# marcinp7/music-style-transfer

Hardware: AMD Instinct MI355X
Metric: style-transfer opt iters/sec (higher is better)
Workload: dtype f32; 1 GPU; one 30 s clip per GPU (BASELINE.json configs[1]): piano-roll C=4,R=16,T=4 (+percussion), full widths (980325 params), fwd+loss+bwd every step, Adam+StepLR every iter_size steps; clips_per_gpu=1, iter_size=2, hip_graph=True, graphs=one joint graph, accumulation=2 concurrent streams, launches_per_pass=71, parallelism=single GPU

## Files before the change

### music-style-transfer_amd/csrc/loss_optim.hip

```cpp
#include "mst_common.h"

#define LOSS_MAXBLK 256
#define NP_SUMS 7
#define N_TAPE_IN 16
#define SAVED_J 0
#define EPS_DIV 1e-7f

int64_t mst_loss_scratch_floats(void) { return 2 * LOSS_MAXBLK * 8 + 64; }

template <int NFEAT>
__device__ __forceinline__ void note_terms(const float* p, const float* t, float* acc) {
    const float pv = p[1], tv = t[1];
    const float m = tv > 0.f ? 1.f : 0.f;
    acc[0] += fminf(pv, tv);
    acc[1] += fmaxf(pv - tv, 0.f);
    acc[2] += fmaxf(tv - pv, 0.f);
    const float dv = tv - pv;
    acc[3] += dv * dv * m;
    const float dd = (p[0] - fminf(t[0], 6.f)) / 6.f;
    acc[4] += dd * dd * m;
    if (NFEAT == 5) {
        float bce = 0.f;
#pragma unroll
        for (int a = 2; a < 5; ++a) {
// ... 112 lines not shown
        o.acc = d_div(in[5], d_cmul(NM, 3.f));
        if (normalize) o.acc = d_tanh(o.acc);
        o.total = d_qmean3(o.dur, o.acc, nv);
    } else {
        o.acc = dl(0.f, 0.f);
        o.total = d_qmean2(o.dur, nv);
    }
    return o;
}

__global__ __launch_bounds__(64) void loss_tail_kernel(const float* scratch, int nblk_p, int nblk_u, int has_u,
                                                       const float* il, const float* it, int ni,
                                                       const float* mlg, const float* mt,
                                                       const float* bp, const float* bt, int normalize,
                                                       float* losses, float* saved, LossBatch lb,
                                                       float* gl_onehot, float* losses_out) {
    __shared__ float sums[N_TAPE_IN];
    const int tid = threadIdx.x;
    {
        const int64_t k = blockIdx.y;
        scratch += k * lb.tmp; il += k * lb.ws; it += k * lb.ws; mlg += k * lb.ws; mt += k * lb.ws; bp += k * lb.ws;
        bt += k * lb.ws; losses += k * lb.ws; saved += k * lb.ws;
        if (gl_onehot) gl_onehot += k * lb.ws;
        if (losses_out) losses_out += k * MST_N_LOSSES;
    }
    {
        float sp[8] = {0.f, 0.f, 0.f, 0.f, 0.f, 0.f, 0.f, 0.f}, su[8] = {0.f, 0.f, 0.f, 0.f, 0.f, 0.f, 0.f, 0.f};
        typedef float row4 __attribute__((ext_vector_type(4), aligned(4)));
        const row4* rp = reinterpret_cast<const row4*>(scratch);
        const row4* ru = reinterpret_cast<const row4*>(scratch + LOSS_MAXBLK * 8);
        const int nbu = has_u ? nblk_u : 0;
        for (int q = tid; q < nblk_p; q += 64) {
            const row4 x = rp[2 * q], y = rp[2 * q + 1];
            sp[0] += x.x; sp[1] += x.y; sp[2] += x.z; sp[3] += x.w; sp[4] += y.x; sp[5] += y.y; sp[6] += y.z;
        }
        for (int q = tid; q < nbu; q += 64) {
            const row4 x = ru[2 * q], y = ru[2 * q + 1];
            su[0] += x.x; su[1] += x.y; su[2] += x.z; su[3] += x.w; su[4] += y.x; su[5] += y.y; su[6] += y.z;
        }
// ... 11 lines not shown
    for (int j = tid; j < ni; j += 64) {
        const float x = il[j];
        v += fmaxf(x, 0.f) - x * it[j] + log1pf(expf(-fabsf(x)));
    }
    v = wave_sum(v);
    if (tid == 0) {
        sums[13] = v / (float)ni;
        const int tgt = mt[1] > mt[0] ? 1 : 0;
        const float mx = fmaxf(mlg[0], mlg[1]);
        const float lse = mx + logf(expf(mlg[0] - mx) + expf(mlg[1] - mx));
        sums[14] = lse - mlg[tgt];
        const float db = (bp[0] - bt[0]) / 150.f;
        sums[15] = db * db;
    }
    __syncthreads();
    if (tid >= N_TAPE_IN) return;
    Dual in[N_TAPE_IN];
#pragma unroll
    for (int j = 0; j < N_TAPE_IN; ++j) in[j] = dl(sums[j], j == tid ? 1.f : 0.f);
    Dual leaf[MST_N_LOSSES];
    bool present[MST_N_LOSSES];
#pragma unroll
    for (int k = 0; k < MST_N_LOSSES; ++k) { leaf[k] = dl(0.f, 0.f); present[k] = true; }
    const ChannelLeaves p = channel_tree(in, true, normalize != 0);
    leaf[MST_L_P_TOTAL] = p.total; leaf[MST_L_P_NOTES] = p.notes; leaf[MST_L_P_VELOCITY] = p.vel;
    leaf[MST_L_P_DURATION] = p.dur; leaf[MST_L_P_ACCIDENTALS] = p.acc;
    if (has_u) {
        const ChannelLeaves u = channel_tree(in + 7, false, normalize != 0);
        leaf[MST_L_U_TOTAL] = u.total; leaf[MST_L_U_NOTES] = u.notes; leaf[MST_L_U_VELOCITY] = u.vel;
        leaf[MST_L_U_DURATION] = u.dur;
        leaf[MST_L_CH_TOTAL] = d_qmean2(p.total, u.total);
    } else {
        present[MST_L_U_TOTAL] = present[MST_L_U_NOTES] = present[MST_L_U_VELOCITY] = present[MST_L_U_DURATION] = false;
        leaf[MST_L_CH_TOTAL] = p.total;
    }
    Dual li = in[13], lm = in[14];
    if (normalize) { li = d_tanh(li); lm = d_tanh(lm); }
    leaf[MST_L_SI_INSTRUMENTS] = li;
    leaf[MST_L_SI_MODE] = lm;
    leaf[MST_L_SI_BPM] = in[15];
    leaf[MST_L_SI_TOTAL] = d_qmean3(li, lm, in[15]);
    leaf[MST_L_TOTAL] = d_qmean2(leaf[MST_L_CH_TOTAL], leaf[MST_L_SI_TOTAL]);
#pragma unroll
    for (int k = 0; k < MST_N_LOSSES; ++k) {
        if (tid == 0) {
            const float v = present[k] ? leaf[k].v : __builtin_nanf("");
            losses[k] = v;
            if (losses_out) losses_out[k] = v;
            if (gl_onehot) gl_onehot[k] = k == MST_L_TOTAL ? 1.f : 0.f;
        }
        saved[SAVED_J + k * N_TAPE_IN + tid] = present[k] ? leaf[k].d : 0.f;
    }
}

__global__ __launch_bounds__(256) void loss_bwd_kernel(const float* pp, const float* pt, int64_t np, int nblk_p,
                                                       const float* up, const float* ut, int64_t nu, int nblk_u,
                                                       const float* il, const float* it, int ni,
                                                       const float* mlg, const float* mt, const float* bp, const float* bt,
                                                       const float* saved, const float* gl,
                                                       float* gp, float* gu, float* gi, float* gm, float* gb, LossBatch lb, float info_scale) {
    __shared__ float coef[N_TAPE_IN];
    __shared__ float tile_p[256 * 5], tile_t[256 * 5];
    {
        const int64_t k = blockIdx.y;
        pp += k * lb.ws; pt += k * lb.ext0; up += k * lb.ws; ut += k * lb.ext1;
        il += k * lb.ws; it += k * lb.ws; mlg += k * lb.ws; mt += k * lb.ws; bp += k * lb.ws; bt += k * lb.ws;
// ... 33 lines not shown
#pragma unroll
                for (int u = 0; u < 5; ++u) {
                    const int j = min((int)threadIdx.x + 256 * u, cnt - 1);
                    pv[u] = Pg[j]; tv[u] = Tg[j];
                }
#pragma unroll
                for (int u = 0; u < 5; ++u) {
                    const int j = threadIdx.x + 256 * u;
                    if (j < cnt) { tile_p[j] = pv[u]; tile_t[j] = tv[u]; }
                }
            }
            __syncthreads();
            if ((int)threadIdx.x < rows) {
                float* p = tile_p + threadIdx.x * nf;
                const float* t = tile_t + threadIdx.x * nf;
                const float pv = p[1], tv = t[1], p0 = p[0];
                const float m = tv > 0.f ? 1.f : 0.f;
                float gv = cTP * (pv < tv ? 1.f : (pv == tv ? 0.5f : 0.f));
                gv += cFP * (pv - tv > 0.f ? 1.f : 0.f) - cFN * (tv - pv > 0.f ? 1.f : 0.f);
                gv -= cSEV * 2.f * (tv - pv) * m;
                p[1] = gv;
                p[0] = cSED * 2.f * (p0 - fminf(t[0], 6.f)) * (1.f / 36.f) * m;
                if (pitched) {
#pragma unroll
                    for (int a = 2; a < 5; ++a)
                        p[a] = cBCE * m * (p[a] - t[a]) / fmaxf((1.f - p[a]) * p[a], 1e-12f);
                }
            }
            __syncthreads();
#pragma unroll
            for (int u = 0; u < 5; ++u) {
                const int j = threadIdx.x + 256 * u;
                if (j < cnt) Gg[j] = tile_p[j];
            }
            __syncthreads();
        }
    } else {
// ... 7 lines not shown
            gm[1] = cm * (e1 / (e0 + e1) - (tgt == 1 ? 1.f : 0.f));
            gb[0] = cb * 2.f * (bp[0] - bt[0]) / (150.f * 150.f);
        }
    }
}

static int blocks_for(int64_t n) {
    int64_t b = (n + 1023) / 1024;
    if (b < 1) b = 1;
    if (b > LOSS_MAXBLK) b = LOSS_MAXBLK;
    return (int)b;
}

int loss_fwd_batched(const float* pp, const float* pt, int64_t np, const float* up, const float* ut, int64_t nu, const float* il,
                     const float* it, int ni, const float* mlg, const float* mt, const float* bp, const float* bt, int normalize,
                     float* losses, float* saved, float* scratch, LossBatch lb, hipStream_t s, float* gl_onehot, float* losses_out) {
    if (!pp || !pt || !il || !it || !mlg || !mt || !bp || !bt || !losses || !saved || !scratch || np <= 0 || lb.clips < 1)
        return MST_ERR_ARG;
    const int has_u = (up && ut && nu > 0) ? 1 : 0;
    const int nbp = blocks_for(np), nbu = has_u ? blocks_for(nu) : 0;
    hipLaunchKernelGGL(loss_partials_kernel, dim3(nbp + nbu, lb.clips), dim3(256), 0, s, pp, pt, np, nbp, up, ut,
                       has_u ? nu : (int64_t)0, nbu, scratch, lb);
    hipLaunchKernelGGL(loss_tail_kernel, dim3(1, lb.clips), dim3(64), 0, s, (const float*)scratch, nbp, nbu, has_u, il, it,
                       ni, mlg, mt, bp, bt, normalize, losses, saved, lb, gl_onehot, losses_out);
    return hipGetLastError() == hipSuccess ? MST_OK : MST_ERR_LAUNCH;
}

int loss_bwd_batched(const float* pp, const float* pt, int64_t np, const float* up, const float* ut, int64_t nu, const float* il,
                     const float* it, int ni, const float* mlg, const float* mt, const float* bp, const float* bt,
                     const float* saved, const float* gl, float* gp, float* gu, float* gi, float* gm, float* gb, LossBatch lb,
                     hipStream_t s, float info_scale) {
    if (!pp || !pt || !saved || !gl || !gi || !gm || !gb || np <= 0 || lb.clips < 1) return MST_ERR_ARG;
    const int has_u = (up && ut && gu && nu > 0) ? 1 : 0;
    const int nbp = gp ? blocks_for(np) : 0, nbu = has_u ? blocks_for(nu) : 0;
    hipLaunchKernelGGL(loss_bwd_kernel, dim3(nbp + nbu + 1, lb.clips), dim3(256), 0, s, pp, pt, np, nbp, up, ut,
                       has_u ? nu : (int64_t)0, nbu, il, it, ni, mlg, mt, bp, bt, saved, gl, gp, gu, gi, gm, gb, lb, info_scale);
    return hipGetLastError() == hipSuccess ? MST_OK : MST_ERR_LAUNCH;
}

// ... 3 lines not shown

int loss_fwd_partials(const float* pp, const float* pt, int64_t np, const float* up, const float* ut, int64_t nu, float* scratch,
                      hipStream_t s) {
    const int has_u = (up && ut && nu > 0) ? 1 : 0;
    const int nbp = blocks_for(np), nbu = has_u ? blocks_for(nu) : 0;
    hipLaunchKernelGGL(loss_partials_kernel, dim3(nbp + nbu, 1), dim3(256), 0, s, pp, pt, np, nbp, up, ut,
                       has_u ? nu : (int64_t)0, nbu, scratch, ONE_CLIP);
    return hipGetLastError() == hipSuccess ? MST_OK : MST_ERR_LAUNCH;
}

int loss_fwd_tail(int64_t np, int64_t nu, int has_u, const float* il, const float* it, int ni, const float* mlg, const float* mt,
                  const float* bp, const float* bt, int normalize, float* losses, float* saved, float* scratch, hipStream_t s,
                  float* gl_onehot, float* losses_out) {
    const int nbp = blocks_for(np), nbu = has_u ? blocks_for(nu) : 0;
    hipLaunchKernelGGL(loss_tail_kernel, dim3(1, 1), dim3(64), 0, s, (const float*)scratch, nbp, nbu, has_u, il, it,
                       ni, mlg, mt, bp, bt, normalize, losses, saved, ONE_CLIP, gl_onehot, losses_out);
    return hipGetLastError() == hipSuccess ? MST_OK : MST_ERR_LAUNCH;
}

extern "C" int32_t mst_total_loss_fwd(const float* pp, const float* pt, int64_t np, const float* up, const float* ut,
                                      int64_t nu, const float* il, const float* it, int32_t ni, const float* mlg,
                                      const float* mt, const float* bp, const float* bt, int32_t normalize,
                                      float* losses, float* saved, float* scratch, mst_stream stream) {
    return loss_fwd_batched(pp, pt, np, up, ut, nu, il, it, (int)ni, mlg, mt, bp, bt, (int)normalize, losses, saved, scratch,
                            ONE_CLIP, (hipStream_t)stream, nullptr, nullptr);
}

extern "C" int32_t mst_total_loss_bwd(const float* pp, const float* pt, int64_t np, const float* up, const float* ut,
                                      int64_t nu, const float* il, const float* it, int32_t ni, const float* mlg,
                                      const float* mt, const float* bp, const float* bt, const float* saved,
                                      const float* gl, float* gp, float* gu, float* gi, float* gm, float* gb,
// ... 990 lines not shown
```

### music-style-transfer_amd/csrc/mst_common.h

```cpp
#pragma once
#include <hip/hip_runtime.h>
#include <stdint.h>

#include "../../include/mst_amd.h"

#ifndef MST_GLOBAL_AS
#define MST_GLOBAL_AS __attribute__((address_space(1)))
#endif
#ifndef MST_CONST_AS
#define MST_CONST_AS __attribute__((address_space(4)))
#endif
#ifndef MST_UNIFORM
#define MST_UNIFORM(x) __builtin_amdgcn_readfirstlane(x)
#endif
#ifndef MST_FAST_EXP
#define MST_FAST_EXP(x) __expf(x)
#define MST_FAST_RCP(x) __builtin_amdgcn_rcpf(x)
#define MST_PIN(x) asm volatile("" : "+v"(x))
#endif
#ifndef MST_PIN_SGPR
#if defined(__AMDGCN__)
#define MST_PIN_SGPR(p) asm volatile("" : "+s"(p))
#else
#define MST_PIN_SGPR(p) ((void)(p))
// ... 15 lines not shown
#endif

#define NF 10
#define NPF 5
#define NUF 2
#define NOCT 8
#define NDEG 7
#define NPN 56
#define NUN 47
#define CONV_K 14
#define CONV_PAD 4
#define LEAKY 0.01f

enum { SP_WS = 0, SP_PAR = 1, SP_GPAR = 2, SP_EXT0 = 3, SP_EXT1 = 4, SP_GRAD = 5, SP_TMP = 6, SP_COUNT = 7 };
enum { MST_BF_LOSS_FUSED = 1,
       MST_BF_ALL_STAGES = 2 };
struct Bases { float* p[SP_COUNT]; int32_t flags; };

enum { ACT_NONE = 0, ACT_LEAKY = 1, ACT_SIGOUT = 2, ACT_BPM = 3 };

enum { OPK_DENSE = 0, OPK_ACTGRAD = 2, OPK_IM2COL = 3, OPK_PERMW = 4, OPK_CONVGRAD = 5 };
#define MAX_SEG 6
struct Seg {
    int32_t space, ld, start, width;
    int64_t off;
    int32_t s[4];
};
struct Operand {
    int32_t kind;
    int32_t space;
    int64_t off;
// ... 168 lines not shown
    int64_t w_off, b_off;
    int64_t slab_off, slab_stride, rows_per_split; int32_t splits;
    int32_t first[2];
};
int launch_lin_fwd(const LinDesc& d, Bases b, hipStream_t s);
int launch_lin_dx(const LinDesc& d, Bases b, int first, hipStream_t s);
int launch_lin_dw(const LinDesc& d, Bases b, hipStream_t s);
int lin_dw_tiles(const LinDesc& d);

struct RowLinDesc {
    int32_t rows, kin, nout, act, xgrad;
    int64_t x_off, y_off;
    int64_t w_off, b_off;
    int64_t slab_off; int32_t slab_stride, nblk;
    int32_t first;
};

struct CopyDesc { int64_t src_off, dst_off; int32_t na, nb, cols, src_sa, src_sb, dst_sa, dst_sb, first; };
struct FoldDesc { int32_t space, nrows, row_stride, ncols, col_stride, pad; int64_t part_off, sum_off ; };
int launch_copy_rows(const CopyDesc* dev, const CopyDesc& host, int backward, Bases b, hipStream_t s);
int launch_fold(const FoldDesc* dev, int spread, Bases b, hipStream_t s);
int launch_combine_phase(const CombineDesc* dev, int nblk, int which, Bases b, hipStream_t s, int count = 1, int mc4 = 0, int whole_small = 0);

struct SlabEntry { int64_t dst, src, stride; int32_t count, splits; int32_t reps; int64_t rep_stride; int32_t width, dst_ld; int32_t single;
                   int64_t base;  };
struct SlabBlock { int32_t entry, start; };

struct Sizes {
    int OC, PCE_IL, H, HB;
    int SE_L, SE_IL, SE_ML, SE_BL;
// ... 17 lines not shown
int launch_segred2(const SegRedDesc* dev_descs, int count, int stage2_blocks, Bases b, hipStream_t s);
int launch_lstm_transpose(const LstmDesc* dev_descs, int count, int maxH, int multi, Bases b, hipStream_t s);
int launch_lstm_fwd(const LstmDesc* dev_descs, int count, int maxB, int maxH, int multi, int small, Bases b, hipStream_t s);
int launch_lstm_bwd(const LstmDesc* dev_descs, int count, int maxB, int maxH, int multi, int small, Bases b, hipStream_t s);
bool lstm_small(int count, int maxB, int maxH);
int lstm_multi_blocks_per_cu();
int launch_combine_fwd(const CombineDesc* dev_descs, int count, int max_nblk, int all_small, int mc4, Bases b, hipStream_t s);
int launch_combine_bwd(const CombineDesc* dev_descs, int count, int max_nblk, int all_small, int mc4, Bases b, hipStream_t s);
int launch_me_sumsq(const NotesDesc* dev, const NotesDesc& host, int count, Bases b, hipStream_t s);
int launch_me_notes_fwd(const NotesDesc* dev, const NotesDesc& host, int count, Bases b, hipStream_t s);
int launch_me_bwd_reduce(const NotesDesc* dev, const NotesDesc& host, int count, Bases b, hipStream_t s);
int launch_me_notes_bwd(const NotesDesc* dev, const NotesDesc& host, int count, Bases b, hipStream_t s);
int launch_psa_notes_fwd(const NotesDesc* dev, const NotesDesc& host, int count, Bases b, hipStream_t s);
int launch_psa_notes_bwd(const NotesDesc* dev, const NotesDesc& host, int count, Bases b, hipStream_t s);
int psa_bwd_waves(int C);
struct LossBatch { int32_t clips; int64_t ws, grad, tmp, ext0, ext1; };
int loss_fwd_partials(const float* pp, const float* pt, int64_t np, const float* up, const float* ut, int64_t nu, float* scratch,
                      hipStream_t s);
int loss_fwd_tail(int64_t np, int64_t nu, int has_u, const float* il, const float* it, int ni, const float* mlg, const float* mt,
                  const float* bp, const float* bt, int normalize, float* losses, float* saved, float* scratch, hipStream_t s,
                  float* gl_onehot, float* losses_out);
int loss_blocks(int64_t n);
int loss_fwd_batched(const float* pp, const float* pt, int64_t np, const float* up, const float* ut, int64_t nu, const float* il,
                     const float* it, int ni, const float* mlg, const float* mt, const float* bp, const float* bt, int normalize,
                     float* losses, float* saved, float* scratch, LossBatch lb, hipStream_t s,
                     float* gl_onehot ,
                     float* losses_out );
int loss_bwd_batched(const float* pp, const float* pt, int64_t np, const float* up, const float* ut, int64_t nu, const float* il,
                     const float* it, int ni, const float* mlg, const float* mt, const float* bp, const float* bt,
                     const float* saved, const float* gl, float* gp, float* gu, float* gi, float* gm, float* gb, LossBatch lb,
                     hipStream_t s, float info_scale = 1.f );
int launch_roll_metrics(const float* pred, const float* target, int64_t n_groups, int64_t group_cells, int nfeat, int gpc,
                        int64_t pred_cs, int64_t tgt_cs, void* scratch, hipStream_t s);
struct EvalMetricsArgs {
    const void* part_p; int64_t slices_p, cells_p;
    const void* part_u; int64_t slices_u, cells_u;
    int32_t C, ni;
    const float *il, *it, *mlg, *mt, *bp, *bt;
    int64_t ws_stride;
    double* out;
};
int launch_eval_metrics_finish(const EvalMetricsArgs& a, int clips, hipStream_t s);
// ... 14 lines not shown
```

### music-style-transfer_amd/csrc/notes.hip

```cpp
#include "mst_common.h"

__device__ __forceinline__ float lrelu(float z) { return z > 0.f ? z : z * LEAKY; }
__device__ __forceinline__ float dlrelu(float y) { return y > 0.f ? 1.f : LEAKY; }

typedef float nt_f32x4 __attribute__((ext_vector_type(4)));
#define NT_ROW 66

__device__ __forceinline__ float wave_sum64(float v) {
#pragma unroll
    for (int o = 32; o > 0; o >>= 1) v += __shfl_xor(v, o);
    return v;
}

template <int N>
__device__ __forceinline__ void ld_vec(const float* p, float (&v)[N]) {
    static_assert(N % 4 == 0, "16-byte rows");
#pragma unroll
    for (int i = 0; i < N / 4; ++i) { const float4 t = reinterpret_cast<const float4*>(p)[i]; v[4 * i] = t.x; v[4 * i + 1] = t.y; v[4 * i + 2] = t.z; v[4 * i + 3] = t.w; }
}
template <int N>
__device__ __forceinline__ void st_vec(float* p, const float (&v)[N]) {
#pragma unroll
    for (int i = 0; i < N / 4; ++i) reinterpret_cast<float4*>(p)[i] = make_float4(v[4 * i], v[4 * i + 1], v[4 * i + 2], v[4 * i + 3]);
}
// ... 840 lines not shown
    float* y0 = b.p[SP_WS] + d.y_off;
    for (int row = blockIdx.x * 256 + tid; row < d.rows; row += gridDim.x * 256) {
        float x[KIN], y[NOUT];
        rl_load<KIN>(x0 + (int64_t)row * KIN, x);
#pragma unroll
        for (int n = 0; n < NOUT; ++n) {
            float z = b_s[n];
#pragma unroll
            for (int k = 0; k < KIN; ++k) z = fmaf(w_s[n * KIN + k], x[k], z);
            y[n] = rl_act(d.act, z, n);
        }
        rl_store<NOUT>(y0 + (int64_t)row * NOUT, y);
    }
}

template <int KIN, int NOUT>
__global__ __launch_bounds__(256) void rowlin_bwd_kernel(const RowLinDesc* __restrict__ dp, Bases b) {
    const RowLinDesc d = dp[blockIdx.y];
    constexpr int NACC = NOUT * KIN + NOUT;
    constexpr int RW = NOUT + KIN;
    constexpr int RP = 256 + 4;
    static_assert(NACC <= 256, "role count exceeds the workgroup");
    __shared__ float w_s[NOUT * KIN];
    __shared__ __attribute__((aligned(16))) float st[RW][RP];
    const int tid = threadIdx.x;
    for (int i = tid; i < NOUT * KIN; i += 256) w_s[i] = b.p[SP_PAR][d.w_off + i];
    const float* x0 = b.p[SP_WS] + d.x_off;
    const float* y0 = b.p[SP_WS] + d.y_off;
    const float* gy0 = b.p[SP_GRAD] + d.y_off;
    float* gx0 = b.p[SP_GRAD] + d.x_off;
    const int rn = tid < NOUT * KIN ? tid / KIN : tid - NOUT * KIN;
    const int rk = tid < NOUT * KIN ? NOUT + tid % KIN : -1;
    float wacc = 0.f;
    for (int base = blockIdx.x * 256; base < d.rows; base += gridDim.x * 256) {
        const int row = base + tid;
        __syncthreads();
        if (row < d.rows) {
            float x[KIN], y[NOUT], g[NOUT];
            rl_load<KIN>(x0 + (int64_t)row * KIN, x);
            rl_load<NOUT>(y0 + (int64_t)row * NOUT, y);
            rl_load<NOUT>(gy0 + (int64_t)row * NOUT, g);
#pragma unroll
            for (int n = 0; n < NOUT; ++n) { g[n] *= rl_dact(d.act, y[n], n); st[n][tid] = g[n]; }
#pragma unroll
            for (int k = 0; k < KIN; ++k) st[NOUT + k][tid] = x[k];
            if (d.xgrad) {
                float dx[KIN];
                if (d.first) {
#pragma unroll
                    for (int k = 0; k < KIN; ++k) dx[k] = 0.f;
                } else rl_load<KIN>(gx0 + (int64_t)row * KIN, dx);
#pragma unroll
                for (int k = 0; k < KIN; ++k) {
                    float a = 0.f;
#pragma unroll
                    for (int n = 0; n < NOUT; ++n) a = fmaf(g[n], w_s[n * KIN + k], a);
// ... 29 lines not shown
bool rowlin_supported(int kin, int nout) { return (kin == 8 && nout == 20) || (kin == 4 && nout == 14) || (kin == 8 && nout == 2); }

#define ROWLIN_DISPATCH(KERN, GRID)                                                                         \
    if (h.kin == 8 && h.nout == 20) hipLaunchKernelGGL((KERN<8, 20>), GRID, dim3(256), 0, s, dev, b);         \
    else if (h.kin == 4 && h.nout == 14) hipLaunchKernelGGL((KERN<4, 14>), GRID, dim3(256), 0, s, dev, b);    \
    else if (h.kin == 8 && h.nout == 2) hipLaunchKernelGGL((KERN<8, 2>), GRID, dim3(256), 0, s, dev, b);      \
    else return MST_ERR_UNSUPPORTED;

int launch_rowlin_fwd(const RowLinDesc* dev, const RowLinDesc& h, int count, Bases b, hipStream_t s) {
    int nb = (h.rows + 255) / 256;
    if (nb > 1024) nb = 1024;
    ROWLIN_DISPATCH(rowlin_fwd_kernel, dim3(nb, count));
    return (int)hipGetLastError();
}
int launch_rowlin_bwd(const RowLinDesc* dev, const RowLinDesc& h, int count, Bases b, hipStream_t s) {
    ROWLIN_DISPATCH(rowlin_bwd_kernel, dim3(h.nblk, count));
    return (int)hipGetLastError();
}
```

### music-style-transfer_amd/csrc/plan.hip

```cpp
#include <cmath>
#include <cstdio>
#include <cstdlib>
#include <cstring>
#include <map>
#include <string>
#include <array>
#include <vector>

#include "mst_common.h"

#define MST_ALIGN_UP(n) (((n) + 63) / 64 * 64)

static int mean_size(double a, double b, double factor = 1.0) { return (int)std::ceil(((a + b) / 2.0) * factor); }

Sizes mst_sizes(const mst_dims& d) {
    Sizes z{};
    z.I = d.instr; z.STYLE = d.style; z.BAR = d.bar; z.H = d.beat; z.HB = d.bar / 2; z.RH = d.rhythm;
    z.MEL = d.melody; z.NRF = d.nrf; z.NI = d.n_instruments;
    z.OC = mean_size(NF * NPF, d.beat);
    z.PCE_IL = mean_size(d.instr, d.beat);
    z.SE_L = mean_size(d.bar, d.style);
    z.SE_IL = mean_size(d.instr, d.style, .25);
    z.SE_ML = mean_size(2, d.style, .1);
    z.SE_BL = mean_size(d.style, 1, .05);
// ... 236 lines not shown
    mst_plan_options opt{};
    int mfma = 0;
    int lstm_small_on = 1;

    bool tiled() const { return opt.tile_rows > 0; }
    bool mixes() const { return !mfma && !tiled() && opt.branches != 1 && !opt.no_merge; }
    int mc4() const { return d.C <= 4 ? 1 : 0; }
    int Rl() const { return tiled() ? opt.tile_rows : d.R; }
    int P() const { return d.C * Rl() * d.T; }
    int Q() const { return Rl() * d.T; }
    struct Xchg { int space; int64_t off; int32_t len; };
    std::vector<Xchg> xchgs;
    bool tags_in_zero = false;
    int zero_ride = -1;
    void find_zero_ride();
    std::vector<ZeroChunk> zero_fwd; ZeroChunk* d_zero_fwd = nullptr;
    int64_t loss_sum_off = 0;
    int loss_fold[2] = {-1, -1};
    struct Phase { int what; int pass; int begin, end; int nx; int xchg[MST_MAX_XCHG]; };
    std::vector<Phase> phases;
    int K() const { return d.clips > 1 ? d.clips : 1; }
    static int device_cus() {
#ifdef HIPSIM
        return 16;
#else
        int dev = 0, cus = 0;
        if (hipGetDevice(&dev) != hipSuccess || hipDeviceGetAttribute(&cus, hipDeviceAttributeMultiprocessorCount, dev) != hipSuccess) return 0;
        return cus;
#endif
    }
// ... 57 lines not shown
        return r;
    }
    LstmDesc reloc(LstmDesc l, int k) const {
        const int64_t a = shift(SP_WS, k), t = shift(SP_TMP, k);
        l.zx_off += a; l.out_off += a; l.gout_off += a; l.gzx_off += a;
        l.gates_off += t; l.c_off += t; l.hprev_off += t; l.tc_off += t; l.xch_off += t;
        return l;
    }
    CombineDesc reloc(CombineDesc c, int k) const {
        const int64_t a = shift(SP_WS, k), t = shift(SP_TMP, k);
        c.x_off += a; c.out_off += a; c.gx_off += a; c.gout_off += a; c.stats_off += t; c.part_off += t;
        return c;
    }
    RowLinDesc reloc(RowLinDesc r, int k) const {
        r.x_off += shift(SP_WS, k); r.y_off += shift(SP_WS, k); r.slab_off += shift(SP_TMP, k);
        return r;
    }
    NotesDesc reloc(NotesDesc n, int k) const {
        const int64_t a = shift(SP_WS, k), t = shift(SP_TMP, k);
        n.oct_off += a; n.deg_off += a; n.rt_oct_off += a; n.rt_deg_off += a; n.it_oct_off += a; n.it_deg_off += a; n.mel_off += a; n.g_mel_off += a; n.out_off += a; n.g_out_off += a; n.g_oct_off += a; n.g_deg_off += a;
        n.g_ml_off += a; n.x_off += shift(n.x_space, k); n.slab_off += t; n.part_off += t; n.stats_off += t;
        n.itp_oct_off += a; n.itp_deg_off += a; n.loss_saved_off += a; n.loss_gl_off += a;
        return n;
    }
    template <class F> void with_sched_table(int fam, F&& f) {
        switch (fam) {
        case F_GEMM: f(gemms); break;       case F_GATHER: f(gathers); break;     case F_SEGRED: f(segreds); break;
        case F_LSTM: f(lstms); break;       case F_COMB: f(combines); break;      case F_NOTES: f(notes); break;
        case F_ROWLIN: f(rowlins); break;   default: err = MST_ERR_UNSUPPORTED;
        }
// ... 650 lines not shown
        Op op; op.stage = AP;
        op.fwd.push_back(Step{K_PSA_F, (int)notes.host.size(), 1, 0, 0});
        op.bwd.push_back(Step{K_PSA_B, (int)notes.host.size(), 1, 0, 0});
        notes.host.push_back(n); ops.push_back(op);
        slabs[2].push_back(SlabEntry{n.wm_off, n.slab_off, nw, nw, n.nblk});
    }
    if (U) {
        m = "unpitched_style_applier";
        T usa_sl = linear(AP, style, true, m + ".style_linear", NF * z.USA_SL, ACT_LEAKY);
        T usa_rl = linear(AP, rhythm, true, m + ".rhythm_linear", z.USA_RL, ACT_LEAKY);
        T sl_view{usa_sl.off, NF, z.USA_SL, z.USA_SL};
        const int rsQ_F[4] = {Q_, NF, 1, 1};
        T ucat = gather(AP, rsQ_F, {seg(sl_view, 0, 1, 0, 0), seg(usa_rl, NF, 1, 0, 0)});
        T v = linear(AP, ucat, true, m + ".notes_linear", NUN * NUF * 4, ACT_LEAKY);
        T v_rows{v.off, Q_ * NF * NUN, NUF * 4, NUF * 4};
        rowlin(AP, v_rows, true, m + ".linear", NUF, ACT_SIGOUT, "unpitched_pred");
    }
    if (!widths_supported(z)) err = MST_ERR_UNSUPPORTED;
}

static void acc_add(std::vector<Acc>& v, int space, int64_t lo, int64_t len, bool w, bool accum = false, bool dense = true) {
    if (space != SP_WS && space != SP_GRAD && space != SP_TMP) return;
    if (len <= 0) return;
    Acc a{space, lo, lo + len, w}; a.accum = accum; a.dense = dense;
    v.push_back(a);
}

static void operand_acc(std::vector<Acc>& v, const Operand& o, int di, int dj, int ones) {
    switch (o.kind) {
    case OPK_DENSE: {
        const int64_t si = o.si < 0 ? -o.si : o.si, sj = o.sj < 0 ? -o.sj : o.sj;
// ... 816 lines not shown
        return launch_slab_reduce(p->d_slabs_all, p->d_slab_blocks_all, (int)p->slab_blocks_all.size(), b, (hipStream_t)stream) ? MST_ERR_LAUNCH : MST_OK;
    for (int s = 2; s >= 0; --s) {
        if (!((mask >> s) & 1)) continue;
        if (launch_slab_reduce(p->d_slabs[s], p->d_slab_blocks[s], (int)p->slab_blocks[s].size(), b, (hipStream_t)stream))
            return MST_ERR_LAUNCH;
    }
    return MST_OK;
}

extern "C" int32_t mst_backward(const mst_plan* p, int32_t mask, const float* params, float* gparams, float* ws,
                                const float* pitched, const float* unpitched, mst_stream stream) {
    return backward_impl(p, mask, params, gparams, ws, pitched, unpitched, stream, 0);
}

enum { LOSS_WHOLE, LOSS_PARTIALS, LOSS_TAIL };
static int loss_forward(const mst_plan* p, int what, float* ws, const float* pitched, const float* unpitched, float* losses, hipStream_t st) {
    const mst_plan::LossOps& o = p->loss;
    const bool U = p->d.has_unpitched != 0;
    const float *pp = ws + o.pp, *up = U ? ws + o.up : nullptr, *ut = U ? unpitched : nullptr;
    float* scratch = ws + p->arena(SP_TMP) + p->loss_scratch;
    if (what == LOSS_PARTIALS) return loss_fwd_partials(pp, pitched, o.np, up, ut, o.nu, scratch, st);
    if (what == LOSS_TAIL)
        return loss_fwd_tail(o.np, o.nu, U ? 1 : 0, ws + o.il, ws + o.it, p->z.NI, ws + o.mlg, ws + o.mt, ws + o.bp, ws + o.bt, 1,
                             ws + o.losses, ws + o.saved, scratch, st, ws + o.gl, losses);
    return loss_fwd_batched(pp, pitched, o.np, up, ut, o.nu, ws + o.il, ws + o.it, p->z.NI, ws + o.mlg, ws + o.mt, ws + o.bp, ws + o.bt, 1,
                            ws + o.losses, ws + o.saved, scratch, p->loss_batch(), st, ws + o.gl, losses);
}
static int loss_backward(const mst_plan* p, float* ws, const float* pitched, const float* unpitched, bool pitched_grad, const LossBatch& lb,
                         float info_scale, hipStream_t st) {
    const mst_plan::LossOps& o = p->loss;
    const bool U = p->d.has_unpitched != 0;
    float* g = ws + p->arena(SP_GRAD);
    return loss_bwd_batched(ws + o.pp, pitched, o.np, U ? ws + o.up : nullptr, U ? unpitched : nullptr, o.nu, ws + o.il, ws + o.it, p->z.NI,
                            ws + o.mlg, ws + o.mt, ws + o.bp, ws + o.bt, ws + o.saved, ws + o.gl, pitched_grad ? g + o.pp : nullptr,
                            U ? g + o.up : nullptr, g + o.il, g + o.mlg, g + o.bp, lb, st, info_scale);
}

extern "C" int32_t mst_train_iteration(const mst_plan* p, const float* params, float* gparams, float* ws,
                                       const float* pitched, const float* unpitched, float* losses, mst_stream stream) {
    if (!p || !params || !gparams || !ws || !pitched) return MST_ERR_ARG;
    hipStream_t st = (hipStream_t)stream;
    int e = p->zero_ride >= 0 ? 0 : mst_zero_grads(p, MST_STAGE_ALL, ws, stream);
    if (e) return e;
    if (p->d.has_unpitched && !unpitched) return MST_ERR_ARG;
    e = run_pass(p, p->list(MST_STAGE_ALL, 0), MST_STAGE_ALL, make_bases(p, params, nullptr, ws, pitched, unpitched), st, p->tags_in_zero, p->zero_ride);
    if (e) return e;
    e = loss_forward(p, LOSS_WHOLE, ws, pitched, unpitched, losses, st);
    if (e) return e;
    e = loss_backward(p, ws, pitched, unpitched, false , p->loss_batch(), 1.f, st);
    if (e) return e;
    e = backward_impl(p, MST_STAGE_ALL, params, gparams, ws, pitched, unpitched, stream, MST_BF_LOSS_FUSED);
    if (e) return e;
    return hipGetLastError() == hipSuccess ? MST_OK : MST_ERR_LAUNCH;
}

static int64_t eval_slices(const mst_plan* p, bool pitched) {
    return mst_roll_slices(pitched ? (int64_t)p->Q() * NF * NPN : (int64_t)p->Q() * NF * NUN);
}

extern "C" int64_t mst_eval_scratch_bytes(const mst_plan* p) {
    if (!p) return MST_ERR_ARG;
    if (p->tiled()) return MST_ERR_UNSUPPORTED;
    return 32 * (int64_t)p->K() * ((int64_t)p->d.C * eval_slices(p, true) + (p->d.has_unpitched ? eval_slices(p, false) : 0));
}

extern "C" int32_t mst_eval_iteration(const mst_plan* p, const float* params, float* ws, const float* pitched,
// ... 227 lines not shown
    int n = 0;
    for (int q = 0; q < s.b && n < cap; ++q, ++n) {
        const GemmDesc& g = p->gemms.sched[s.first + q];
        int32_t* o = out + 6 * n;
        o[0] = g.M; o[1] = g.N; o[2] = g.K; o[3] = g.ksplit; o[4] = g.fold_rows; o[5] = gemm_blocks(g, p->mfma);
    }
    return n;
}

extern "C" int32_t mst_plan_time_steps(const mst_plan* p, int32_t mask, int32_t backward, const float* params, float* gparams,
                                       float* ws, const float* pitched, const float* unpitched, mst_stream stream,
                                       int32_t reps, float* ms, int32_t* kind, double* flops, double* bytes) {
    if (!p || !params || !ws || !ms || !kind || !flops || !bytes || reps < 1) return MST_ERR_ARG;
    hipStream_t st = (hipStream_t)stream;
    Bases b = make_bases(p, params, gparams, ws, pitched, unpitched);
    if (backward && !p->tiled()) b.flags = MST_BF_LOSS_FUSED;
    if ((mask & MST_STAGE_ALL) == MST_STAGE_ALL) b.flags |= MST_BF_ALL_STAGES;
    hipEvent_t e0, e1;
    if (hipEventCreate(&e0) != hipSuccess || hipEventCreate(&e1) != hipSuccess) return MST_ERR_ALLOC;
    const std::vector<Step>& L = p->list(mask, backward);
    int idx = 0;
    for (const Step* s : steps_of(p, mask, backward)) {
        float t = 0.f;
        if (s->carrier < 0) {
            run_step(p, L, *s, b, st);
            hipEventRecord(e0, st);
            for (int r = 0; r < reps; ++r) run_step(p, L, *s, b, st);
            hipEventRecord(e1, st);
            hipEventSynchronize(e1);
            hipEventElapsedTime(&t, e0, e1);
        }
// ... 10 lines not shown
```

Measured before the change: 2845 iters/s.

## Fuse loss backward into loss tail and unpitched rowlin backward kernels

The separate loss_backward launch is removed when the loss can be fused. The head gradients (instruments BCE, mode CE, BPM) are now computed in the loss tail kernel. The unpitched-prediction gradient is computed inline in the rowlin backward kernel from the saved loss coefficients and targets. This saves a kernel launch and a full pass over the prediction/target tensors, at the cost of a more complex rowlin kernel and new plan descriptor fields. It relies on the pitched loss gradient already being fused elsewhere via MST_BF_LOSS_FUSED.

Measured after the change: 2872 iters/s, median of 6. Within noise of the previous version (+0.9%).

```diff
diff --git a/music-style-transfer_amd/csrc/loss_optim.hip b/music-style-transfer_amd/csrc/loss_optim.hip
--- a/music-style-transfer_amd/csrc/loss_optim.hip
+++ b/music-style-transfer_amd/csrc/loss_optim.hip
@@ -2,7 +2,7 @@
 
 #define LOSS_MAXBLK 256
 #define NP_SUMS 7
-#define N_TAPE_IN 16
+#define N_TAPE_IN MST_LOSS_TAPE_IN
 #define SAVED_J 0
 #define EPS_DIV 1e-7f
 
@@ -150,8 +150,9 @@
                                                        const float* mlg, const float* mt,
                                                        const float* bp, const float* bt, int normalize,
                                                        float* losses, float* saved, LossBatch lb,
-                                                       float* gl_onehot, float* losses_out) {
+                                                       float* gl_onehot, float* losses_out, LossHeadGrads hg) {
     __shared__ float sums[N_TAPE_IN];
+    __shared__ float head_coef[3];
     const int tid = threadIdx.x;
     {
         const int64_t k = blockIdx.y;
@@ -159,6 +160,7 @@
         bt += k * lb.ws; losses += k * lb.ws; saved += k * lb.ws;
         if (gl_onehot) gl_onehot += k * lb.ws;
         if (losses_out) losses_out += k * MST_N_LOSSES;
+        if (hg.gi) { hg.gi += k * lb.grad; hg.gm += k * lb.grad; hg.gb += k * lb.grad; }
     }
     {
         float sp[8] = {0.f, 0.f, 0.f, 0.f, 0.f, 0.f, 0.f, 0.f}, su[8] = {0.f, 0.f, 0.f, 0.f, 0.f, 0.f, 0.f, 0.f};
@@ -200,42 +202,56 @@
         sums[15] = db * db;
     }
     __syncthreads();
-    if (tid >= N_TAPE_IN) return;
-    Dual in[N_TAPE_IN];
-#pragma unroll
-    for (int j = 0; j < N_TAPE_IN; ++j) in[j] = dl(sums[j], j == tid ? 1.f : 0.f);
-    Dual leaf[MST_N_LOSSES];
-    bool present[MST_N_LOSSES];
-#pragma unroll
-    for (int k = 0; k < MST_N_LOSSES; ++k) { leaf[k] = dl(0.f, 0.f); present[k] = true; }
-    const ChannelLeaves p = channel_tree(in, true, normalize != 0);
-    leaf[MST_L_P_TOTAL] = p.total; leaf[MST_L_P_NOTES] = p.notes; leaf[MST_L_P_VELOCITY] = p.vel;
-    leaf[MST_L_P_DURATION] = p.dur; leaf[MST_L_P_ACCIDENTALS] = p.acc;
-    if (has_u) {
-        const ChannelLeaves u = channel_tree(in + 7, false, normalize != 0);
-        leaf[MST_L_U_TOTAL] = u.total; leaf[MST_L_U_NOTES] = u.notes; leaf[MST_L_U_VELOCITY] = u.vel;
-        leaf[MST_L_U_DURATION] = u.dur;
-        leaf[MST_L_CH_TOTAL] = d_qmean2(p.total, u.total);
-    } else {
-        present[MST_L_U_TOTAL] = present[MST_L_U_NOTES] = present[MST_L_U_VELOCITY] = present[MST_L_U_DURATION] = false;
-        leaf[MST_L_CH_TOTAL] = p.total;
-    }
-    Dual li = in[13], lm = in[14];
-    if (normalize) { li = d_tanh(li); lm = d_tanh(lm); }
-    leaf[MST_L_SI_INSTRUMENTS] = li;
-    leaf[MST_L_SI_MODE] = lm;
-    leaf[MST_L_SI_BPM] = in[15];
-    leaf[MST_L_SI_TOTAL] = d_qmean3(li, lm, in[15]);
-    leaf[MST_L_TOTAL] = d_qmean2(leaf[MST_L_CH_TOTAL], leaf[MST_L_SI_TOTAL]);
-#pragma unroll
-    for (int k = 0; k < MST_N_LOSSES; ++k) {
-        if (tid == 0) {
-            const float v = present[k] ? leaf[k].v : __builtin_nanf("");
-            losses[k] = v;
-            if (losses_out) losses_out[k] = v;
-            if (gl_onehot) gl_onehot[k] = k == MST_L_TOTAL ? 1.f : 0.f;
-        }
-        saved[SAVED_J + k * N_TAPE_IN + tid] = present[k] ? leaf[k].d : 0.f;
+    if (tid < N_TAPE_IN) {
+        Dual in[N_TAPE_IN];
+#pragma unroll
+        for (int j = 0; j < N_TAPE_IN; ++j) in[j] = dl(sums[j], j == tid ? 1.f : 0.f);
+        Dual leaf[MST_N_LOSSES];
+        bool present[MST_N_LOSSES];
+#pragma unroll
+        for (int k = 0; k < MST_N_LOSSES; ++k) { leaf[k] = dl(0.f, 0.f); present[k] = true; }
+        const ChannelLeaves p = channel_tree(in, true, normalize != 0);
+        leaf[MST_L_P_TOTAL] = p.total; leaf[MST_L_P_NOTES] = p.notes; leaf[MST_L_P_VELOCITY] = p.vel;
+        leaf[MST_L_P_DURATION] = p.dur; leaf[MST_L_P_ACCIDENTALS] = p.acc;
+        if (has_u) {
+            const ChannelLeaves u = channel_tree(in + 7, false, normalize != 0);
+            leaf[MST_L_U_TOTAL] = u.total; leaf[MST_L_U_NOTES] = u.notes; leaf[MST_L_U_VELOCITY] = u.vel;
+            leaf[MST_L_U_DURATION] = u.dur;
+            leaf[MST_L_CH_TOTAL] = d_qmean2(p.total, u.total);
+        } else {
+            present[MST_L_U_TOTAL] = present[MST_L_U_NOTES] = present[MST_L_U_VELOCITY] = present[MST_L_U_DURATION] = false;
+            leaf[MST_L_CH_TOTAL] = p.total;
+        }
+        Dual li = in[13], lm = in[14];
+        if (normalize) { li = d_tanh(li); lm = d_tanh(lm); }
+        leaf[MST_L_SI_INSTRUMENTS] = li;
+        leaf[MST_L_SI_MODE] = lm;
+        leaf[MST_L_SI_BPM] = in[15];
+        leaf[MST_L_SI_TOTAL] = d_qmean3(li, lm, in[15]);
+        leaf[MST_L_TOTAL] = d_qmean2(leaf[MST_L_CH_TOTAL], leaf[MST_L_SI_TOTAL]);
+#pragma unroll
+        for (int k = 0; k < MST_N_LOSSES; ++k) {
+            if (tid == 0) {
+                const float v = present[k] ? leaf[k].v : __builtin_nanf("");
+                losses[k] = v;
+                if (losses_out) losses_out[k] = v;
+                if (gl_onehot) gl_onehot[k] = k == MST_L_TOTAL ? 1.f : 0.f;
+            }
+            saved[SAVED_J + k * N_TAPE_IN + tid] = present[k] ? leaf[k].d : 0.f;
+        }
+        if (hg.gi && tid >= 13) head_coef[tid - 13] = 0.f + leaf[MST_L_TOTAL].d;
+    }
+    if (!hg.gi) return;
+    __syncthreads();
+    const float ci = head_coef[0], cm = head_coef[1], cb = head_coef[2];
+    for (int j = tid; j < ni; j += 64) hg.gi[j] = ci * (1.f / (1.f + expf(-il[j])) - it[j]) / (float)ni;
+    if (tid == 0) {
+        const int tgt = mt[1] > mt[0] ? 1 : 0;
+        const float mx = fmaxf(mlg[0], mlg[1]);
+        const float e0 = expf(mlg[0] - mx), e1 = expf(mlg[1] - mx);
+        hg.gm[0] = cm * (e0 / (e0 + e1) - (tgt == 0 ? 1.f : 0.f));
+        hg.gm[1] = cm * (e1 / (e0 + e1) - (tgt == 1 ? 1.f : 0.f));
+        hg.gb[0] = cb * 2.f * (bp[0] - bt[0]) / (150.f * 150.f);
     }
 }
 
@@ -299,13 +315,12 @@
             if ((int)threadIdx.x < rows) {
                 float* p = tile_p + threadIdx.x * nf;
                 const float* t = tile_t + threadIdx.x * nf;
-                const float pv = p[1], tv = t[1], p0 = p[0];
+                const float tv = t[1];
                 const float m = tv > 0.f ? 1.f : 0.f;
-                float gv = cTP * (pv < tv ? 1.f : (pv == tv ? 0.5f : 0.f));
-                gv += cFP * (pv - tv > 0.f ? 1.f : 0.f) - cFN * (tv - pv > 0.f ? 1.f : 0.f);
-                gv -= cSEV * 2.f * (tv - pv) * m;
+                float g0, gv;
+                loss_note_grad(p[0], p[1], t[0], tv, cTP, cFP, cFN, cSEV, cSED, g0, gv);
                 p[1] = gv;
-                p[0] = cSED * 2.f * (p0 - fminf(t[0], 6.f)) * (1.f / 36.f) * m;
+                p[0] = g0;
                 if (pitched) {
 #pragma unroll
                     for (int a = 2; a < 5; ++a)
@@ -343,15 +358,17 @@
 
 int loss_fwd_batched(const float* pp, const float* pt, int64_t np, const float* up, const float* ut, int64_t nu, const float* il,
                      const float* it, int ni, const float* mlg, const float* mt, const float* bp, const float* bt, int normalize,
-                     float* losses, float* saved, float* scratch, LossBatch lb, hipStream_t s, float* gl_onehot, float* losses_out) {
+                     float* losses, float* saved, float* scratch, LossBatch lb, hipStream_t s, float* gl_onehot, float* losses_out,
+                     LossHeadGrads hg) {
     if (!pp || !pt || !il || !it || !mlg || !mt || !bp || !bt || !losses || !saved || !scratch || np <= 0 || lb.clips < 1)
         return MST_ERR_ARG;
+    if (hg.gi && (!hg.gm || !hg.gb || !gl_onehot)) return MST_ERR_ARG;
     const int has_u = (up && ut && nu > 0) ? 1 : 0;
     const int nbp = blocks_for(np), nbu = has_u ? blocks_for(nu) : 0;
     hipLaunchKernelGGL(loss_partials_kernel, dim3(nbp + nbu, lb.clips), dim3(256), 0, s, pp, pt, np, nbp, up, ut,
                        has_u ? nu : (int64_t)0, nbu, scratch, lb);
     hipLaunchKernelGGL(loss_tail_kernel, dim3(1, lb.clips), dim3(64), 0, s, (const float*)scratch, nbp, nbu, has_u, il, it,
-                       ni, mlg, mt, bp, bt, normalize, losses, saved, lb, gl_onehot, losses_out);
+                       ni, mlg, mt, bp, bt, normalize, losses, saved, lb, gl_onehot, losses_out, hg);
     return hipGetLastError() == hipSuccess ? MST_OK : MST_ERR_LAUNCH;
 }
 
@@ -385,7 +402,7 @@
                   float* gl_onehot, float* losses_out) {
     const int nbp = blocks_for(np), nbu = has_u ? blocks_for(nu) : 0;
     hipLaunchKernelGGL(loss_tail_kernel, dim3(1, 1), dim3(64), 0, s, (const float*)scratch, nbp, nbu, has_u, il, it,
-                       ni, mlg, mt, bp, bt, normalize, losses, saved, ONE_CLIP, gl_onehot, losses_out);
+                       ni, mlg, mt, bp, bt, normalize, losses, saved, ONE_CLIP, gl_onehot, losses_out, LossHeadGrads{nullptr, nullptr, nullptr});
     return hipGetLastError() == hipSuccess ? MST_OK : MST_ERR_LAUNCH;
 }
 
diff --git a/music-style-transfer_amd/csrc/mst_common.h b/music-style-transfer_amd/csrc/mst_common.h
--- a/music-style-transfer_amd/csrc/mst_common.h
+++ b/music-style-transfer_amd/csrc/mst_common.h
@@ -53,7 +53,8 @@
 
 enum { SP_WS = 0, SP_PAR = 1, SP_GPAR = 2, SP_EXT0 = 3, SP_EXT1 = 4, SP_GRAD = 5, SP_TMP = 6, SP_COUNT = 7 };
 enum { MST_BF_LOSS_FUSED = 1,
-       MST_BF_ALL_STAGES = 2 };
+       MST_BF_ALL_STAGES = 2,
+       MST_BF_LOSS_ROWLIN = 4 };
 struct Bases { float* p[SP_COUNT]; int32_t flags; };
 
 enum { ACT_NONE = 0, ACT_LEAKY = 1, ACT_SIGOUT = 2, ACT_BPM = 3 };
@@ -252,6 +253,8 @@
     int64_t w_off, b_off;
     int64_t slab_off; int32_t slab_stride, nblk;
     int32_t first;
+    int32_t loss, t_space;
+    int64_t t_off, loss_saved_off;
 };
 
 struct CopyDesc { int64_t src_off, dst_off; int32_t na, nb, cols, src_sa, src_sb, dst_sa, dst_sb, first; };
@@ -299,18 +302,30 @@
 int launch_psa_notes_fwd(const NotesDesc* dev, const NotesDesc& host, int count, Bases b, hipStream_t s);
 int launch_psa_notes_bwd(const NotesDesc* dev, const NotesDesc& host, int count, Bases b, hipStream_t s);
 int psa_bwd_waves(int C);
+#define MST_LOSS_TAPE_IN 16
+__device__ __forceinline__ void loss_note_grad(float p0, float pv, float t0, float tv, float cTP, float cFP, float cFN, float cSEV,
+                                               float cSED, float& g0, float& gv) {
+    const float m = tv > 0.f ? 1.f : 0.f;
+    float g = cTP * (pv < tv ? 1.f : (pv == tv ? 0.5f : 0.f));
+    g += cFP * (pv - tv > 0.f ? 1.f : 0.f) - cFN * (tv - pv > 0.f ? 1.f : 0.f);
+    g -= cSEV * 2.f * (tv - pv) * m;
+    gv = g;
+    g0 = cSED * 2.f * (p0 - fminf(t0, 6.f)) * (1.f / 36.f) * m;
+}
 struct LossBatch { int32_t clips; int64_t ws, grad, tmp, ext0, ext1; };
 int loss_fwd_partials(const float* pp, const float* pt, int64_t np, const float* up, const float* ut, int64_t nu, float* scratch,
                       hipStream_t s);
 int loss_fwd_tail(int64_t np, int64_t nu, int has_u, const float* il, const float* it, int ni, const float* mlg, const float* mt,
                   const float* bp, const float* bt, int normalize, float* losses, float* saved, float* scratch, hipStream_t s,
                   float* gl_onehot, float* losses_out);
+struct LossHeadGrads { float *gi, *gm, *gb; };
 int loss_blocks(int64_t n);
 int loss_fwd_batched(const float* pp, const float* pt, int64_t np, const float* up, const float* ut, int64_t nu, const float* il,
                      const float* it, int ni, const float* mlg, const float* mt, const float* bp, const float* bt, int normalize,
                      float* losses, float* saved, float* scratch, LossBatch lb, hipStream_t s,
                      float* gl_onehot ,
-                     float* losses_out );
+                     float* losses_out ,
+                     LossHeadGrads hg = LossHeadGrads{nullptr, nullptr, nullptr} );
 int loss_bwd_batched(const float* pp, const float* pt, int64_t np, const float* up, const float* ut, int64_t nu, const float* il,
                      const float* it, int ni, const float* mlg, const float* mt, const float* bp, const float* bt,
                      const float* saved, const float* gl, float* gp, float* gu, float* gi, float* gm, float* gb, LossBatch lb,
diff --git a/music-style-transfer_amd/csrc/notes.hip b/music-style-transfer_amd/csrc/notes.hip
--- a/music-style-transfer_amd/csrc/notes.hip
+++ b/music-style-transfer_amd/csrc/notes.hip
@@ -878,21 +878,28 @@
     }
 }
 
-template <int KIN, int NOUT>
+template <int KIN, int NOUT, bool LOSS>
 __global__ __launch_bounds__(256) void rowlin_bwd_kernel(const RowLinDesc* __restrict__ dp, Bases b) {
     const RowLinDesc d = dp[blockIdx.y];
+    static_assert(!LOSS || NOUT == NUF, "the loss flavour is the unpitched prediction's");
     constexpr int NACC = NOUT * KIN + NOUT;
     constexpr int RW = NOUT + KIN;
     constexpr int RP = 256 + 4;
     static_assert(NACC <= 256, "role count exceeds the workgroup");
-    __shared__ float w_s[NOUT * KIN];
+    __shared__ float w_s[NOUT * KIN + (LOSS ? 5 : 0)];
     __shared__ __attribute__((aligned(16))) float st[RW][RP];
+    float* const coef_s = w_s + NOUT * KIN;
     const int tid = threadIdx.x;
     for (int i = tid; i < NOUT * KIN; i += 256) w_s[i] = b.p[SP_PAR][d.w_off + i];
     const float* x0 = b.p[SP_WS] + d.x_off;
     const float* y0 = b.p[SP_WS] + d.y_off;
-    const float* gy0 = b.p[SP_GRAD] + d.y_off;
+    float* gy0 = b.p[SP_GRAD] + d.y_off;
     float* gx0 = b.p[SP_GRAD] + d.x_off;
+    const float* t0 = nullptr;
+    if (LOSS) {
+        if (tid < 5) coef_s[tid] = 0.f + b.p[SP_WS][d.loss_saved_off + MST_L_TOTAL * MST_LOSS_TAPE_IN + 7 + tid];
+        t0 = b.p[d.t_space] + d.t_off;
+    }
     const int rn = tid < NOUT * KIN ? tid / KIN : tid - NOUT * KIN;
     const int rk = tid < NOUT * KIN ? NOUT + tid % KIN : -1;
     float wacc = 0.f;
@@ -903,7 +910,12 @@
             float x[KIN], y[NOUT], g[NOUT];
             rl_load<KIN>(x0 + (int64_t)row * KIN, x);
             rl_load<NOUT>(y0 + (int64_t)row * NOUT, y);
-            rl_load<NOUT>(gy0 + (int64_t)row * NOUT, g);
+            if constexpr (LOSS) {
+                float t[NOUT];
+                rl_load<NOUT>(t0 + (int64_t)row * NOUT, t);
+                loss_note_grad(y[0], y[1], t[0], t[1], coef_s[0], coef_s[1], coef_s[2], coef_s[3], coef_s[4], g[0], g[1]);
+                rl_store<NOUT>(gy0 + (int64_t)row * NOUT, g);
+            } else rl_load<NOUT>(gy0 + (int64_t)row * NOUT, g);
 #pragma unroll
             for (int n = 0; n < NOUT; ++n) { g[n] *= rl_dact(d.act, y[n], n); st[n][tid] = g[n]; }
 #pragma unroll
@@ -963,6 +975,14 @@
     return (int)hipGetLastError();
 }
 int launch_rowlin_bwd(const RowLinDesc* dev, const RowLinDesc& h, int count, Bases b, hipStream_t s) {
-    ROWLIN_DISPATCH(rowlin_bwd_kernel, dim3(h.nblk, count));
+    if (h.loss && (b.flags & MST_BF_LOSS_ROWLIN)) {
+        if (h.kin != 8 || h.nout != NUF) return MST_ERR_UNSUPPORTED;
+        hipLaunchKernelGGL((rowlin_bwd_kernel<8, NUF, true>), dim3(h.nblk, count), dim3(256), 0, s, dev, b);
+        return (int)hipGetLastError();
+    }
+    if (h.kin == 8 && h.nout == 20) hipLaunchKernelGGL((rowlin_bwd_kernel<8, 20, false>), dim3(h.nblk, count), dim3(256), 0, s, dev, b);
+    else if (h.kin == 4 && h.nout == 14) hipLaunchKernelGGL((rowlin_bwd_kernel<4, 14, false>), dim3(h.nblk, count), dim3(256), 0, s, dev, b);
+    else if (h.kin == 8 && h.nout == 2) hipLaunchKernelGGL((rowlin_bwd_kernel<8, 2, false>), dim3(h.nblk, count), dim3(256), 0, s, dev, b);
+    else return MST_ERR_UNSUPPORTED;
     return (int)hipGetLastError();
 }
diff --git a/music-style-transfer_amd/csrc/plan.hip b/music-style-transfer_amd/csrc/plan.hip
--- a/music-style-transfer_amd/csrc/plan.hip
+++ b/music-style-transfer_amd/csrc/plan.hip
@@ -274,6 +274,8 @@
     bool tags_in_zero = false;
     int zero_ride = -1;
     void find_zero_ride();
+    bool loss_rowlin = false;
+    bool loss_fused() const { return !tiled() && !opt.no_merge && (!d.has_unpitched || loss_rowlin); }
     std::vector<ZeroChunk> zero_fwd; ZeroChunk* d_zero_fwd = nullptr;
     int64_t loss_sum_off = 0;
     int loss_fold[2] = {-1, -1};
@@ -361,6 +363,7 @@
     }
     RowLinDesc reloc(RowLinDesc r, int k) const {
         r.x_off += shift(SP_WS, k); r.y_off += shift(SP_WS, k); r.slab_off += shift(SP_TMP, k);
+        if (r.loss) { r.t_off += shift(r.t_space, k); r.loss_saved_off += shift(SP_WS, k); }
         return r;
     }
     NotesDesc reloc(NotesDesc n, int k) const {
@@ -1041,7 +1044,13 @@
         T ucat = gather(AP, rsQ_F, {seg(sl_view, 0, 1, 0, 0), seg(usa_rl, NF, 1, 0, 0)});
         T v = linear(AP, ucat, true, m + ".notes_linear", NUN * NUF * 4, ACT_LEAKY);
         T v_rows{v.off, Q_ * NF * NUN, NUF * 4, NUF * 4};
+        const size_t sites = rowlins.host.size();
         rowlin(AP, v_rows, true, m + ".linear", NUF, ACT_SIGOUT, "unpitched_pred");
+        if (rowlins.host.size() > sites) {
+            RowLinDesc& r = rowlins.host.back();
+            r.loss = 1; r.t_space = SP_EXT1; r.t_off = 0; r.loss_saved_off = t_saved.off;
+            loss_rowlin = true;
+        }
     }
     if (!widths_supported(z)) err = MST_ERR_UNSUPPORTED;
 }
@@ -1888,17 +1897,20 @@
 }
 
 enum { LOSS_WHOLE, LOSS_PARTIALS, LOSS_TAIL };
-static int loss_forward(const mst_plan* p, int what, float* ws, const float* pitched, const float* unpitched, float* losses, hipStream_t st) {
+static int loss_forward(const mst_plan* p, int what, float* ws, const float* pitched, const float* unpitched, float* losses, hipStream_t st,
+                        bool head_grads = false) {
     const mst_plan::LossOps& o = p->loss;
     const bool U = p->d.has_unpitched != 0;
     const float *pp = ws + o.pp, *up = U ? ws + o.up : nullptr, *ut = U ? unpitched : nullptr;
     float* scratch = ws + p->arena(SP_TMP) + p->loss_scratch;
+    float* g = ws + p->arena(SP_GRAD);
     if (what == LOSS_PARTIALS) return loss_fwd_partials(pp, pitched, o.np, up, ut, o.nu, scratch, st);
     if (what == LOSS_TAIL)
         return loss_fwd_tail(o.np, o.nu, U ? 1 : 0, ws + o.il, ws + o.it, p->z.NI, ws + o.mlg, ws + o.mt, ws + o.bp, ws + o.bt, 1,
                              ws + o.losses, ws + o.saved, scratch, st, ws + o.gl, losses);
     return loss_fwd_batched(pp, pitched, o.np, up, ut, o.nu, ws + o.il, ws + o.it, p->z.NI, ws + o.mlg, ws + o.mt, ws + o.bp, ws + o.bt, 1,
-                            ws + o.losses, ws + o.saved, scratch, p->loss_batch(), st, ws + o.gl, losses);
+                            ws + o.losses, ws + o.saved, scratch, p->loss_batch(), st, ws + o.gl, losses,
+                            head_grads ? LossHeadGrads{g + o.il, g + o.mlg, g + o.bp} : LossHeadGrads{nullptr, nullptr, nullptr});
 }
 static int loss_backward(const mst_plan* p, float* ws, const float* pitched, const float* unpitched, bool pitched_grad, const LossBatch& lb,
                          float info_scale, hipStream_t st) {
@@ -1919,11 +1931,14 @@
     if (p->d.has_unpitched && !unpitched) return MST_ERR_ARG;
     e = run_pass(p, p->list(MST_STAGE_ALL, 0), MST_STAGE_ALL, make_bases(p, params, nullptr, ws, pitched, unpitched), st, p->tags_in_zero, p->zero_ride);
     if (e) return e;
-    e = loss_forward(p, LOSS_WHOLE, ws, pitched, unpitched, losses, st);
+    const bool fused = p->loss_fused();
+    e = loss_forward(p, LOSS_WHOLE, ws, pitched, unpitched, losses, st, fused);
     if (e) return e;
-    e = loss_backward(p, ws, pitched, unpitched, false , p->loss_batch(), 1.f, st);
-    if (e) return e;
-    e = backward_impl(p, MST_STAGE_ALL, params, gparams, ws, pitched, unpitched, stream, MST_BF_LOSS_FUSED);
+    if (!fused) {
+        e = loss_backward(p, ws, pitched, unpitched, false , p->loss_batch(), 1.f, st);
+        if (e) return e;
+    }
+    e = backward_impl(p, MST_STAGE_ALL, params, gparams, ws, pitched, unpitched, stream, MST_BF_LOSS_FUSED | (fused ? MST_BF_LOSS_ROWLIN : 0));
     if (e) return e;
     return hipGetLastError() == hipSuccess ? MST_OK : MST_ERR_LAUNCH;
 }
@@ -2181,7 +2196,7 @@
     if (!p || !params || !ws || !ms || !kind || !flops || !bytes || reps < 1) return MST_ERR_ARG;
     hipStream_t st = (hipStream_t)stream;
     Bases b = make_bases(p, params, gparams, ws, pitched, unpitched);
-    if (backward && !p->tiled()) b.flags = MST_BF_LOSS_FUSED;
+    if (backward && !p->tiled()) b.flags = MST_BF_LOSS_FUSED | (p->loss_fused() ? MST_BF_LOSS_ROWLIN : 0);
     if ((mask & MST_STAGE_ALL) == MST_STAGE_ALL) b.flags |= MST_BF_ALL_STAGES;
     hipEvent_t e0, e1;
     if (hipEventCreate(&e0) != hipSuccess || hipEventCreate(&e1) != hipSuccess) return MST_ERR_ALLOC;
```
